# UoB-HPC/neutral

Hardware: AMD Instinct MI355X
Metric: particle-steps/sec (higher is better)
Workload: dtype f64

## Files before the change

neutral_amd/csrc/neutral_abi.hip:

```cpp
#include "neutral_abi_state.h"

#include <utility>

using namespace neutral_abi;


namespace {

struct StageMs {
  double kernel = 0.0, sort = 0.0, stream = 0.0, collide = 0.0, exported = 0.0, exchange = 0.0;
};

struct Step {
  neutral::SolveArgs a = {};
  neutral::StepOptions options;
  bool tiled = false;
  bool decomposed = false;
  bool exchange = false;
  bool pass_export = false;
  bool checked = false;
  State::Store* shard = nullptr;
  neutral::StepCounters hc[2] = {};
  unsigned long long check[8] = {0};
  unsigned ctrl[16] = {0};
// ... 47 lines not shown
      HIP_CHECK(hipEventElapsedTime(&ms, g.ev_start, g.ev_streamed));
    }
    stage.stream += (double)ms;
    HIP_CHECK(hipEventElapsedTime(&ms, g.ev_streamed, g.ev_collected));
    stage.sort += (double)ms;
    HIP_CHECK(hipEventElapsedTime(&ms, g.ev_collected, g.ev_stop));
    stage.collide += (double)ms;
  } else {
    stage.collide += (double)ms;
  }
  HIP_CHECK(hipEventElapsedTime(&ms, g.ev_stop, g.ev_exported));
  stage.exported += (double)ms;
  if (s.exchange) {
    HIP_CHECK(hipEventElapsedTime(&ms, g.ev_exchange_begins, g.ev_exchanged));
    stage.exchange += (double)ms;
  }
}

void export_records_by_id(const Step& s, const int* abort_flag) {
  const neutral::SolveArgs& a = s.a;
  HIP_CHECK(neutral::launch_export_records(
      g.tiled.rec_out, g.tiled.slot_of_id, a.p, a.nparticles, g.stream, abort_flag,
      a.export_skip_long_dead ? neutral::tiled_first_inactive(g.tiled) : nullptr, 0xFFFFFFFFu,
      nullptr, 0, a.export_skip_long_dead != 0));
}

void run_batch(Step& s, const BatchSpec& spec) {
  neutral::SolveArgs& a = s.a;
  HIP_CHECK(hipEventRecord(g.ev_start, g.stream));
  if (s.tiled) {
    HIP_CHECK(neutral::launch_solve_tiled(a, s.options, g.tiled, g.stream, spec.plan, spec.first_pass,
                                          spec.first_sort_timed ? g.ev_sorted : nullptr, g.ev_streamed,
                                          g.ev_collected, &s.passes, spec.split));
  } else {
    HIP_CHECK(neutral::launch_solve(a, s.options, g.variant, g.stream));
  }
  HIP_CHECK(hipEventRecord(g.ev_stop, g.stream));
  if (s.exchange) {
    exchange_step(a, s.tiled);
  } else {
    tallies_to_caller(a);
  }
  if (spec.split) {
    HIP_CHECK(neutral::launch_split_export(a, g.tiled, *spec.split, g.ev_collected));
    HIP_CHECK(hipStreamWaitEvent(g.stream, g.ev_split_done, 0));
  } else if (s.pass_export && !s.decomposed) {
    export_records_by_id(s, spec.guarded ? a.abort_flag : nullptr);
// ... 668 lines not shown
```

neutral_amd/csrc/neutral_history.h:

```cpp
#ifndef NEUTRAL_AMD_HISTORY_H
#define NEUTRAL_AMD_HISTORY_H

#include "neutral_device.h"
#include "neutral_kernels.h"

namespace neutral {

constexpr unsigned kMaxEventsPerHistory = 1u << 27;

enum Event : int {
  kEvEnd = 0,
  kEvFacet = 1,
  kEvCollision = 2,
  kEvCensus = 3,
};

struct History {
  double x, y, omega_x, omega_y, energy, weight, dt_to_census, mfp_to_collision;
  int cellx, celly, dead;
  double local_density, micro_s, micro_a, number_density, macro_s, macro_a, speed;
  double energy_deposition;
  double track_length;
  double u_x_inv, u_y_inv, dep_sigma, dep_heat;
  double r_speed, r_cell_mfp;
// ... 434 lines not shown
  h.id = (unsigned)pid;
}

__device__ __forceinline__ void store_particle_view(const History& h, const ParticleView& p,
                                                    int pid) {
  p.x[pid] = h.x;
  p.y[pid] = h.y;
  p.omega_x[pid] = h.omega_x;
  p.omega_y[pid] = h.omega_y;
  p.energy[pid] = h.energy;
  p.weight[pid] = h.weight;
  p.dt_to_census[pid] = h.dt_to_census;
  p.mfp_to_collision[pid] = h.mfp_to_collision;
  p.cellx[pid] = h.cellx;
  p.celly[pid] = h.celly;
  p.dead[pid] = h.dead;
}

__device__ __forceinline__ void store_particle(const History& h, const SolveArgs& a, int pid) {
  store_particle_view(h, a.p, pid);
}

constexpr int kRecStateBits = 3;
constexpr int kRecChanged = (int)0x80000000u;
constexpr unsigned kIdChanged = 0x80000000u;
__device__ __forceinline__ int record_word(int state, unsigned counter) {
  return state | (int)((counter << kRecStateBits) & 0x7FFFFFFFu);
}
__device__ __forceinline__ int record_state(int word) { return word & ((1 << kRecStateBits) - 1); }
__device__ __forceinline__ unsigned record_counter(int word) {
  return ((unsigned)word & 0x7FFFFFFFu) >> kRecStateBits;
}

__device__ __forceinline__ void load_record(History& h, const SolveArgs& a, const ParticleRec& r,
                                            bool keep_changed = false) {
  h.x = r.x;
  h.y = r.y;
  h.omega_x = r.omega_x;
  h.omega_y = r.omega_y;
  h.energy = r.energy;
  h.weight = r.weight;
  h.dt_to_census = r.dt_to_census;
  h.mfp_to_collision = r.mfp_to_collision;
  h.cellx = r.cellx;
  h.celly = r.celly;
  h.dead = 0;
  h.id = r.id | ((keep_changed && (r.dead & kRecChanged)) ? kIdChanged : 0u);
  h.counter = record_counter(r.dead);
}

enum RecState : int {
  kRecIdle = 0,
  kRecDead = 1,
  kRecCollide = 2,
  kRecMigrate = 3,
  kRecEmigrate = 4,
  kRecGone = 5,
};
constexpr int kReachBits = 2;
constexpr unsigned kSummaryTileMask = (1u << (32 - kRecStateBits - kReachBits)) - 1u;

__device__ __forceinline__ unsigned slot_summary(int state, int cellx, int celly, int tiles_x,
                                                 int tile_shift, unsigned reach = 0u) {
  return ((unsigned)state << (32 - kRecStateBits)) |
         (reach << (32 - kRecStateBits - kReachBits)) |
         ((unsigned)((celly >> tile_shift) * tiles_x + (cellx >> tile_shift)) & kSummaryTileMask);
}
__device__ __forceinline__ unsigned summary_reach(unsigned summary) {
  return (summary >> (32 - kRecStateBits - kReachBits)) & ((1u << kReachBits) - 1u);
}

__device__ __forceinline__ unsigned reach_class(double omega_x, double omega_y, int local_cellx,
                                                int local_celly, int tile_shift, int window_cells,
                                                double cells_per_x, double cells_per_y) {
  const int tile = 1 << tile_shift;
  const int margin = (window_cells - tile) >> 1;
  const int fx = local_cellx & (tile - 1);
  const int fy = local_celly & (tile - 1);
  const double to_edge_x = (double)((omega_x >= 0.0) ? (tile - fx + margin) : (fx + 1 + margin));
  const double to_edge_y = (double)((omega_y >= 0.0) ? (tile - fy + margin) : (fy + 1 + margin));
  const double rate_x = fabs(omega_x) * cells_per_x;
  const double rate_y = fabs(omega_y) * cells_per_y;
  const double path = fmin(to_edge_x / rate_x, to_edge_y / rate_y);
  const double facets = path * (rate_x + rate_y);
  const int cls = (int)(facets * (2.0 / (double)window_cells));
  return (unsigned)((cls < 0) ? 0 : ((cls > 3) ? 3 : cls));
}
__device__ __forceinline__ int summary_state(unsigned summary) {
  return (int)(summary >> (32 - kRecStateBits));
}
__device__ __forceinline__ unsigned summary_tile(unsigned summary) {
  return summary & kSummaryTileMask;
}

__device__ __forceinline__ bool outside_domain(const History& h, const SolveArgs& a) {
  return ((unsigned)(h.cellx - a.x_off) >= (unsigned)a.nx) |
         ((unsigned)(h.celly - a.y_off) >= (unsigned)a.ny);
}

typedef unsigned rec_quad __attribute__((ext_vector_type(4)));
constexpr int kRecQuads = kParticleRecBytes / 16;

__device__ __forceinline__ void record_quads(const History& h, int state, rec_quad (&q)[kRecQuads],
                                             bool changed = false) {
  ParticleRec o;
  o.x = h.x;
  o.y = h.y;
  o.omega_x = h.omega_x;
  o.omega_y = h.omega_y;
  o.energy = h.energy;
  o.weight = h.weight;
  o.dt_to_census = h.dt_to_census;
  o.mfp_to_collision = h.mfp_to_collision;
  o.cellx = h.cellx;
  o.celly = h.celly;
  o.id = h.id & ~kIdChanged;
  o.dead = record_word(state, h.counter) | ((changed || (h.id & kIdChanged)) ? kRecChanged : 0);
  __builtin_memcpy(q, &o, kParticleRecBytes);
}

__device__ __forceinline__ void store_record(const History& h, const SolveArgs& a,
                                             ParticleRec& r, int state, bool changed = false) {
  rec_quad q[kRecQuads];
  record_quads(h, state, q, changed);
  rec_quad* dst = (rec_quad*)__builtin_assume_aligned(&r, 16);
#pragma unroll
  for (int k = 0; k < kRecQuads; ++k) {
    dst[k] = q[k];
  }
}

__device__ __forceinline__ void store_record_through(const History& h, const SolveArgs& a,
                                                     ParticleRec& r, int state) {
  rec_quad q[kRecQuads];
  record_quads(h, state, q);
  static_assert(kRecQuads == 5, "five quads");
  asm volatile(
      "global_store_dwordx4 %0, %1, off sc1\n"
      "global_store_dwordx4 %0, %2, off offset:16 sc1\n"
      "global_store_dwordx4 %0, %3, off offset:32 sc1\n"
      "global_store_dwordx4 %0, %4, off offset:48 sc1\n"
      "global_store_dwordx4 %0, %5, off offset:64 sc1\n"
      "s_nop 1"
      :
      : "v"(&r), "v"(q[0]), "v"(q[1]), "v"(q[2]), "v"(q[3]), "v"(q[4])
      : "memory");
}

__device__ __forceinline__ void drain_stores() { asm volatile("s_waitcnt vmcnt(0)" ::: "memory"); }

__device__ __forceinline__ void load_record_through(History& h, const SolveArgs& a,
                                                    const ParticleRec& r, bool keep_changed = false) {
  rec_quad q[kRecQuads];
  asm volatile(
      "global_load_dwordx4 %0, %5, off sc1\n"
      "global_load_dwordx4 %1, %5, off offset:16 sc1\n"
      "global_load_dwordx4 %2, %5, off offset:32 sc1\n"
      "global_load_dwordx4 %3, %5, off offset:48 sc1\n"
      "global_load_dwordx4 %4, %5, off offset:64 sc1\n"
      "s_waitcnt vmcnt(0)"
      : "=&v"(q[0]), "=&v"(q[1]), "=&v"(q[2]), "=&v"(q[3]), "=&v"(q[4])
      : "v"(&r)
      : "memory");
  ParticleRec o;
  __builtin_memcpy(&o, q, kParticleRecBytes);
  load_record(h, a, o, keep_changed);
}

template <typename T>
__device__ __forceinline__ void load_record_through(History& h, const SolveArgs& a,
                                                    const ParticleRec& r, const T* side, T& side_out) {
  static_assert(sizeof(T) == 16, "one quad");
  rec_quad q[kRecQuads];
  rec_quad s;
  asm volatile(
      "global_load_dwordx4 %0, %6, off sc1\n"
      "global_load_dwordx4 %1, %6, off offset:16 sc1\n"
      "global_load_dwordx4 %2, %6, off offset:32 sc1\n"
      "global_load_dwordx4 %3, %6, off offset:48 sc1\n"
      "global_load_dwordx4 %4, %6, off offset:64 sc1\n"
      "global_load_dwordx4 %5, %7, off sc1\n"
      "s_waitcnt vmcnt(0)"
      : "=&v"(q[0]), "=&v"(q[1]), "=&v"(q[2]), "=&v"(q[3]), "=&v"(q[4]), "=&v"(s)
      : "v"(&r), "v"(side)
      : "memory");
  ParticleRec o;
  __builtin_memcpy(&o, q, kParticleRecBytes);
  load_record(h, a, o);
  __builtin_memcpy(&side_out, &s, 16);
// ... 741 lines not shown
```

neutral_amd/csrc/neutral_kernels.h:

```cpp
#ifndef NEUTRAL_AMD_KERNELS_H
#define NEUTRAL_AMD_KERNELS_H

#include <hip/hip_runtime.h>
#include <stdint.h>

namespace neutral {

struct ParticleView {
  double* x;
  double* y;
  double* omega_x;
  double* omega_y;
  double* energy;
  double* weight;
  double* dt_to_census;
  double* mfp_to_collision;
  int* cellx;
  int* celly;
  int* dead;
};

struct alignas(16) ParticleRec {
  double x, y, dt_to_census, mfp_to_collision;
  int cellx, celly;
  unsigned id;
  int dead;
  double omega_x, omega_y, energy, weight;
};
constexpr int kParticleRecBytes = 80;
static_assert(sizeof(ParticleRec) == kParticleRecBytes, "ParticleRec holds 80 bytes");

struct alignas(16) SuspendExtra {
  double energy_deposition;
  unsigned counter;
  unsigned nevents;
};

struct alignas(16) CarriedStart {
  double micro;
  double minus_log_rn0;
};

struct InjectArgs {
  int nparticles;
  uint64_t pid_base;
  int local_nx;
  int local_ny;
  int pad;
  int x_off;
  int y_off;
  double left_off;
  double bottom_off;
  double width;
// ... 223 lines not shown
hipError_t set_step_options_tiled(const StepOptions& o, hipStream_t stream);
hipError_t launch_solve(const SolveArgs& a, const StepOptions& o, int variant, hipStream_t stream);
hipError_t launch_unphysical_values(const double* v, long long n, unsigned long long* out,
                                    hipStream_t stream);
hipError_t launch_tables_check(const double* ks, const double* vs, int ns, const double* ka,
                               const double* va, int na, unsigned long long expect_hash_s,
                               unsigned long long expect_hash_a, int expect_same,
                               int fast_arithmetic, unsigned long long* out4,
                               hipStream_t stream);


size_t tiled_lds_bytes(const SolveArgs& a, const StepOptions& o, const TiledArgs& t);
hipError_t launch_import_records(const ParticleView& p, ParticleRec* rec, unsigned* info,
                                 unsigned* slot_of_id, unsigned* ids, int tiles_x, int tile_shift,
                                 int x_off, int y_off, int n, hipStream_t stream);
hipError_t launch_refresh_micro(const SolveArgs& a, const TiledArgs& t, hipStream_t stream);
bool tiled_uses_carried(const SolveArgs& a, const TiledArgs& t);
hipError_t launch_export_records(const ParticleRec* rec, const unsigned* slot_of_id,
                                 const ParticleView& p, int n, hipStream_t stream,
                                 const int* abort_flag = nullptr,
                                 const unsigned* first_inactive = nullptr,
                                 unsigned final_from = 0xFFFFFFFFu,
                                 const unsigned* skip_ids = nullptr, int max_blocks = 0,
                                 bool partial_ok = false);
struct SplitExport {
  bool on;
  hipStream_t side;
  hipEvent_t done;
  ParticleView p;
  int skip_long_dead;
};
const unsigned* tiled_first_inactive(const TiledArgs& t);
hipError_t launch_emigrant_count(const TiledArgs& t, int n, const DomainGrid& d, unsigned* counts,
                                 hipStream_t stream);
hipError_t launch_emigrant_pack(const TiledArgs& t, int n, const DomainGrid& d,
                                const unsigned* offset, unsigned* cursor, ParticleRec* send,
                                unsigned* free_slots, unsigned* nfree, hipStream_t stream);
hipError_t launch_immigrant_append(const TiledArgs& t, const ParticleRec* recv, int nrecv,
                                   int first_slot, int x_off, int y_off,
                                   const unsigned* free_slots, int nfree, int reuse,
                                   hipStream_t stream);
hipError_t launch_compact_records(const TiledArgs& t, int n, unsigned* cursor, hipStream_t stream);
hipError_t launch_import_by_slot(const ParticleView& p, const unsigned* keys, const TiledArgs& t,
                                 int x_off, int y_off, int n, hipStream_t stream);
hipError_t launch_export_by_slot(const ParticleRec* rec, const ParticleView& p, unsigned* keys,
                                 int n, hipStream_t stream);
int tiled_tile_shift(int nx, int ny, int nparticles, bool with_flux);
// ... 56 lines not shown
```

neutral_amd/csrc/neutral_kernels.hip:

```cpp
#include "neutral_kernels.h"

#include "neutral_device.h"
#include "neutral_history.h"
#include "neutral_inject.h"
#include "neutral_step_options.h"
#include "neutral_wave.h"

#include <type_traits>

namespace neutral {

constexpr int kBlock = 256;

#define NEUTRAL_COLD_ARGS(a) (kQueue ? cold_args() : (a))


__global__ __launch_bounds__(kBlock) void inject_kernel(InjectArgs a) {
  const int kk = blockIdx.x * kBlock + threadIdx.x;
  if (kk >= a.nparticles) {
    return;
  }
  inject_slot(a, kk, 0, 1.0);
}

// ... 237 lines not shown
  static_assert(sizeof(SolveArgs) % 4 == 0, "SolveArgs is read back word by word");
  union {
    SolveArgs a;
    unsigned w[sizeof(SolveArgs) / 4];
  } u;
#if defined(__HIP_DEVICE_COMPILE__)
  typedef const __attribute__((address_space(4))) unsigned* KernargWords;
  KernargWords p = (KernargWords)__builtin_amdgcn_kernarg_segment_ptr();
  asm volatile("" : "+s"(p));
#pragma unroll
  for (unsigned i = 0; i < sizeof(SolveArgs) / 4; ++i) {
    u.w[i] = p[i];
  }
#else
  __builtin_memset(&u, 0, sizeof(u));
#endif
  return u.a;
}

template <bool kQueue, bool kCarriesMicro = false>
__device__ __forceinline__ void put_back(const History& h, const SolveArgs& a, int pid) {
  if (kQueue) {
    const int state = h.dead ? kRecDead : kRecIdle;
    store_record(h, a, a.rec[pid], state, true);
    a.slot_info[pid] = slot_summary(state, h.cellx - a.x_off, h.celly - a.y_off, a.tiles_x,
                                    a.tile_shift);
    if (kCarriesMicro && a.carried) {
      a.carried[pid].micro = h.micro_s;
    }
    if (a.export_view) {
      const ParticleView* pv = a.export_view;
      asm volatile("" : "+s"(pv));
      store_particle_view(h, *pv, (int)h.id);
    }

  } else {
    store_particle(h, a, pid);
  }
}


template <bool kSameTables, bool kQueue, bool kFlux, bool kChecked, unsigned kScores = 0>
__global__ __launch_bounds__(kBlock, kQueue ? ((kSameTables && !kFlux && !kChecked) ? 4 : 3)
                                             : 3)
void history_regroup_kernel(SolveArgs a) {
  constexpr bool kCollisions = (kScores & kScoreCollisions) != 0;
  constexpr bool kRoulette = (kScores & kScoreRoulette) != 0;
// ... 430 lines not shown
          break;
        }
      }
      if (kQueue) {
        w_ncollisions += (unsigned long long)inner * (unsigned)n_collide;
        if (collides_here) {
          h.nevents += inner;
          if (h.nevents > kMaxEventsPerHistory && want != kWantRefill) {
            atomicAdd(&a.counters->aborted, 1u);
            h.ev = kEvEnd;
            want = kWantStream;
          }
        }
      }
      if (slice_ends) {
        slice = 0;
        const bool out = (want == kWantCollide);
        const unsigned long long m_out = __ballot(out);
        StealWork* const sw = cold_args().steal;
        unsigned readers = __hip_atomic_load(&sw->ring_readers[gw], __ATOMIC_RELAXED, __HIP_MEMORY_SCOPE_AGENT);
        if (out) {
          const SolveArgs c = NEUTRAL_COLD_ARGS(a);
          flush_collision_scores(h, c, tally);
          store_record(h, c, c.rec[pid], kRecCollide);
          SuspendExtra x;
          x.energy_deposition = h.energy_deposition;
          x.counter = h.counter;
          x.nevents = h.nevents;
          c.susp[pid] = x;
          if (kFlux) {
            __hip_atomic_store(&c.susp_track[pid], h.track_length, __ATOMIC_RELAXED, __HIP_MEMORY_SCOPE_AGENT);
          }
          if (kCurrent) {
            double* const pending = d_options.current.susp + 2 * (size_t)pid;
            __hip_atomic_store(&pending[0], h.current_x, __ATOMIC_RELAXED, __HIP_MEMORY_SCOPE_AGENT);
            __hip_atomic_store(&pending[1], h.current_y, __ATOMIC_RELAXED, __HIP_MEMORY_SCOPE_AGENT);
          }
        }
        while (wave_uniform(readers) != 0u) {
          __builtin_amdgcn_s_sleep(1);
          readers = __hip_atomic_load(&sw->ring_readers[gw], __ATOMIC_RELAXED, __HIP_MEMORY_SCOPE_AGENT);
        }
        if (out) {
          __hip_atomic_store(ring_slot(ring_tail + lane_rank(m_out)), (unsigned)pid | kRequeued, __ATOMIC_RELAXED,
                             __HIP_MEMORY_SCOPE_AGENT);
          want = kWantRefill;
        }
        const int n_out = __popcll(m_out);
        w_requeued += (unsigned)n_out;
        drained = false;
        drain_stores();
        unsigned waiting_before = 0;
        if ((threadIdx.x & 63) == 0) {
          waiting_before = (unsigned)atomicAdd(&sw->ring_ctl[gw], (unsigned long long)n_out);
        }
        ring_count = (int)wave_uniform(waiting_before) + n_out;
        ring_tail += n_out;
        ring_tail = (ring_tail >= share) ? ring_tail - share : ring_tail;
      }
    } else {
      if (want == kWantStream) {
        const SolveArgs c = NEUTRAL_COLD_ARGS(a);
        if (h.ev == kEvFacet) {
          nfacets++;
          cross_facet<kChecked>(h, c, tally);
          if (kQueue && c.decomposed && outside_domain(h, c)) {
            store_record(h, c, c.rec[pid], kRecEmigrate);
            c.slot_info[pid] = slot_summary(kRecEmigrate, 0, 0, c.tiles_x, c.tile_shift);
            atomicAdd(c.emigrants, 1u);
            want = kWantRefill;
          } else {
            next_event(true);
            want = (h.ev == kEvCollision) ? kWantCollide : kWantStream;
          }
        } else {
          if (h.ev == kEvCensus) {
            ncensus++;
            census<kChecked>(h, c, tally);
          }
          flush_collision_scores(h, c, tally);
          put_back<kQueue, kSameTables>(h, c, pid);
          want = kWantRefill;
        }
      }
    }
  }
  flush_counters(a, nprocessed, nfacets, ncollisions, ncensus);
  if ((threadIdx.x & 63) == 0) {
    if (w_ncollisions) atomicAdd(&a.counters->ncollisions, w_ncollisions);
    if (w_requeued) atomicAdd(&a.counters->nrequeued, (unsigned long long)w_requeued);
// ... 503 lines not shown
```

neutral_amd/csrc/neutral_tiled.hip:

```cpp
#include <cstdlib>
#include <cstring>
#include <type_traits>

#include "neutral_kernels.h"

#include "neutral_device.h"
#include "neutral_history.h"
#include "neutral_step_options.h"
#include "neutral_wave.h"

namespace neutral {

#ifndef NEUTRAL_STREAM_BLOCK
#define NEUTRAL_STREAM_BLOCK 1024
#endif
constexpr int kStreamBlock = NEUTRAL_STREAM_BLOCK;
constexpr int kChunkParticlesMax = 32768;
constexpr int kChunkParticlesMin = 1024;
constexpr int kStreamRefillMin = 56;
constexpr int kStreamRepeat = 64;
constexpr int kStreamRepeatOnePass = 128;
#ifdef NEUTRAL_NO_CARRIED_START
constexpr bool kCarriedStart = false;
#else
// ... 292 lines not shown
        }
      }
    }
  }
}

__global__ __launch_bounds__(kSortBlock) void import_records_kernel(ParticleView p, ParticleRec* rec,
                                                                    unsigned* info,
                                                                    unsigned* slot_of_id,
                                                                    unsigned* ids, int tiles_x,
                                                                    int tile_shift, int x_off,
                                                                    int y_off, int n) {
  const int i = blockIdx.x * kSortBlock + threadIdx.x;
  if (i < n) {
    ParticleRec r;
    r.x = p.x[i];
    r.y = p.y[i];
    r.omega_x = p.omega_x[i];
    r.omega_y = p.omega_y[i];
    r.energy = p.energy[i];
    r.weight = p.weight[i];
    r.dt_to_census = p.dt_to_census[i];
    r.mfp_to_collision = p.mfp_to_collision[i];
    r.cellx = p.cellx[i];
    r.celly = p.celly[i];
    r.id = (unsigned)i;
    r.dead = p.dead[i];
    rec[i] = r;
    slot_of_id[i] = (unsigned)i;
    ids[i] = (unsigned)i;
    info[i] = slot_summary(r.dead ? kRecDead : kRecIdle, r.cellx - x_off, r.celly - y_off, tiles_x,
                           tile_shift);
  }
}

__global__ __launch_bounds__(kSortBlock) void refresh_micro_kernel(SolveArgs a, TiledArgs t) {
  const long long i = (long long)blockIdx.x * kSortBlock + threadIdx.x;
  if (i >= t.sort_end) {
    return;
  }
  const int state = summary_state(t.info_in[i]);
  if (state == kRecDead || state == kRecGone) {
    return;
  }
  const double energy = t.rec_in[i].energy;
  const int ind = cs_bracket(a.scatter_keys, a.scatter_n, energy);
  t.carried_in[i].micro = a.checked ? cs_interpolate<true>(a.scatter_keys, a.scatter_values, ind, energy)
                            : cs_interpolate<false>(a.scatter_keys, a.scatter_values, ind, energy);
}

__global__ __launch_bounds__(kSortBlock) void export_records_kernel(const ParticleRec* rec,
                                                                    const unsigned* slot_of_id,
                                                                    ParticleView p, int n,
                                                                    const int* abort_flag,
                                                                    const unsigned* first_inactive,
                                                                    unsigned final_from,
                                                                    const unsigned* skip_ids,
                                                                    int partial_ok) {
  if (abort_flag && *abort_flag) {
    return;
  }
  for (long long kk = (long long)blockIdx.x * kSortBlock + threadIdx.x; kk < n; kk += (long long)gridDim.x * kSortBlock) {
    const int k = (int)kk;
    if (skip_ids && ((skip_ids[k >> 5] >> (k & 31)) & 1u)) {
      continue;
    }
    const unsigned slot = slot_of_id[k];
    if (slot >= (first_inactive ? *first_inactive : final_from)) {
      continue;
    }
    const rec_quad* const q = (const rec_quad*)__builtin_assume_aligned(&rec[slot], 16);
    ParticleRec r;
    rec_quad* const rq = (rec_quad*)&r;
    rq[0] = q[0];
    rq[1] = q[1];
    rq[2] = q[2];
    __builtin_nontemporal_store(r.x, &p.x[k]);
    __builtin_nontemporal_store(r.y, &p.y[k]);
    __builtin_nontemporal_store(r.dt_to_census, &p.dt_to_census[k]);
    __builtin_nontemporal_store(r.mfp_to_collision, &p.mfp_to_collision[k]);
    __builtin_nontemporal_store(r.cellx, &p.cellx[k]);
    __builtin_nontemporal_store(r.celly, &p.celly[k]);
    if (!partial_ok || (r.dead & kRecChanged)) {
      rq[3] = q[3];
      rq[4] = q[4];
      __builtin_nontemporal_store(r.omega_x, &p.omega_x[k]);
      __builtin_nontemporal_store(r.omega_y, &p.omega_y[k]);
      __builtin_nontemporal_store(r.energy, &p.energy[k]);
      __builtin_nontemporal_store(r.weight, &p.weight[k]);
      __builtin_nontemporal_store((record_state(r.dead) == kRecDead) ? 1 : 0, &p.dead[k]);
    }
  }
}

__global__ __launch_bounds__(1024) void tile_chunks_kernel(TiledArgs t) {
  __shared__ unsigned s_chunks[1024];
  constexpr int kStagedOffsets = 8192;
  __shared__ unsigned s_offset[kStagedOffsets + 2];
  const int tid = threadIdx.x;
  const bool staged = t.nsort + 1 <= kStagedOffsets;
  if (staged) {
    for (int i = tid; i <= t.nsort + 1; i += 1024) {
      s_offset[i] = t.tile_offset[i];
    }
    __syncthreads();
  }
  const unsigned* offset = staged ? s_offset : t.tile_offset;
  const unsigned nactive = offset[t.nsort];
// ... 525 lines not shown
              unsigned spins = 0;
              do {
                src = __hip_atomic_load(place, __ATOMIC_RELAXED, __HIP_MEMORY_SCOPE_AGENT);
              } while (src == kQueueEmpty && ++spins < (1u << 22));
            } else {
              src = t.order[mine];
            }
            if (src >= (unsigned)a.nparticles) {
              atomicAdd(&a.counters->aborted, 1u);
              ended = true;
            } else {
            pid = fresh ? mine : (int)src;
            double micro = 0.0, minus_log_rn0 = 0.0;
            if (kCarried) {
              const CarriedStart cs = fresh ? t.carried_in[src] : t.carried_out[src];
              micro = cs.micro;
              minus_log_rn0 = cs.minus_log_rn0;
            }
            bool bad_load = false;
            if (from_queue || (queues && !fresh)) {
              load_record_through(h, a, t.rec_out[src], true);
              if (from_queue) {
                const int want_tile = ((h.celly - a.y_off) >> t.tile_shift) * t.tiles_x + ((h.cellx - a.x_off) >> t.tile_shift);
                bad_load = (want_tile != chunk_tile) | (!kDomain && (h.id & ~kIdChanged) >= (unsigned)a.nparticles);
              }
            } else {
              load_record(h, a, fresh ? t.rec_in[src] : t.rec_out[src], !fresh);
            }
            if (fresh) {
              t.id_out[pid] = h.id;
              if (!kDomain && t.slots_by_id) {
                t.slot_of_id[h.id] = (unsigned)pid;
              }
              if (kCarried) {
                t.carried_out[pid].micro = micro;
              }
            }
            if (bad_load) {
              atomicAdd(&a.counters->aborted, 1u);
              ended = true;
            } else {
            if (kCarried) {
              if (fresh) {
                prologue_carried<kChecked>(h, a, micro, minus_log_rn0, uniform_window, window_density);
              } else {
                resume_carried<kChecked>(h, a, micro, uniform_window, window_density);
              }
            } else if (fresh) {
              prologue<kSameTables, kChecked>(h, a, ix);
            } else {
              resume<kSameTables, kChecked>(h, a, ix);
            }
            if (!kDomain) {
              h.counter = 1;
            }
            h.plain_div = 0;
            refresh_speed_reciprocal<kChecked>(h);
            refresh_mfp_reciprocal<kChecked>(h);
            h.dep_rate = deposit_rate(h, a);
// ... 83 lines not shown
            if (!((lx < (unsigned)kW) & (ly < (unsigned)kW)) && far_to_go(h, t)) {
              park = kRecMigrate;
            }
          }
          nfacets += (unsigned)crossed;
          h.nevents += (unsigned)crossed;
          if (!windowed && budget_on && park == kRecIdle && h.ev == kEvFacet &&
              h.nevents >= kUnwindowedBudget) {
            const double ahead = h.speed * h.dt_to_census;
            if (ahead * (fabs(h.omega_x) * t.cells_per_x + fabs(h.omega_y) * t.cells_per_y) >
                kMigrateMinFacets) {
              park = kRecMigrate;
            }
          }
          if (h.nevents > kMaxEventsPerHistory && h.ev == kEvFacet && park == kRecIdle) {
            atomicAdd(&a.counters->aborted, 1u);
            h.ev = kEvEnd;
          }
          PHASE(3);
        } else {
          if (h.ev == kEvCensus) {
            census_streamed<kChecked>(h, a, tally);
          }
          store_record(h, a, t.rec_out[pid], kRecIdle);
          t.info_out[pid] = slot_summary(
              kRecIdle, h.cellx - a.x_off, h.celly - a.y_off, t.tiles_x, t.tile_shift,
              t.reach_classes > 1 ? reach_class(h.omega_x, h.omega_y, h.cellx - a.x_off,
                                                h.celly - a.y_off, t.tile_shift, kW, t.cells_per_x,
                                                t.cells_per_y)
                                  : 0u);
          has = false;
          ended = true;
          did_census = (h.ev == kEvCensus);
          PHASE(6);
        }
      }
      bool queued = false;
      const bool hop = queues && park == kRecMigrate;
      const unsigned long long m_hop = __ballot(hop);
      if (m_hop != 0ull) {
        int dest = 0;
        if (hop) {
          dest = ((h.celly - a.y_off) >> t.tile_shift) * t.tiles_x + ((h.cellx - a.x_off) >> t.tile_shift);
          if ((unsigned)dest >= (unsigned)t.ntiles || (unsigned)pid >= (unsigned)a.nparticles) {
            atomicAdd(&a.counters->aborted, 1u);
            dest = 0;
          }
          store_record_through(h, a, t.rec_out[(unsigned)pid < (unsigned)a.nparticles ? pid : 0], kRecMigrate);
        }
        int leader = -1;
        unsigned rank = 0, group = 0;
        unsigned long long todo = m_hop;
        while (todo != 0ull) {
          const int l = __builtin_ctzll(todo);
          const int tile_l = __builtin_amdgcn_readlane(dest, l);
          const unsigned long long same = __ballot(hop && dest == tile_l);
          if (hop && dest == tile_l) {
            leader = l;
            rank = (unsigned)lane_rank(same);
            group = (unsigned)__popcll(same);
          }
          todo &= ~same;
        }
        drain_stores();
        unsigned base = 0;
        if (hop && leader == (int)(threadIdx.x & 63)) {
          base = atomicAdd(&t.queue_tail[dest], group);
        }
        base = (unsigned)__shfl((int)base, leader < 0 ? 0 : leader, 64);
        if (hop) {
          const unsigned place = base + rank;
          if (place < qcap) {
            __hip_atomic_store(t.queue_entries + ((size_t)dest * qcap + (size_t)place), (unsigned)pid,
                               __ATOMIC_RELAXED, __HIP_MEMORY_SCOPE_AGENT);
            queued = true;
            has = false;
          }
        }
        w_hops += (unsigned)__popcll(__ballot(queued));
        w_overflows += (unsigned)__popcll(__ballot(hop && !queued));
      }
      if (park != kRecIdle && !queued) {
        if (!hop) {
          store_record(h, a, t.rec_out[pid], park);
        }
        t.info_out[pid] = slot_summary(
            park, h.cellx - a.x_off, h.celly - a.y_off, t.tiles_x, t.tile_shift,
            (t.reach_classes > 1 && park == kRecMigrate)
                ? reach_class(h.omega_x, h.omega_y, h.cellx - a.x_off, h.celly - a.y_off,
                              t.tile_shift, kW, t.cells_per_x, t.cells_per_y)
                : 0u);
        has = false;
        ended = true;
      }
      PHASE(7);
      w_ended += (unsigned)__popcll(__ballot(ended));
      w_migrants += (unsigned)__popcll(__ballot(park == kRecMigrate && !queued));
      if (kDomain) {
        w_emigrants += (unsigned)__popcll(__ballot(park == kRecEmigrate));
      }
      w_census += (unsigned)__popcll(__ballot(did_census));
    }
  }
  PHASE(0);
  PHASE_REPORT
  if ((threadIdx.x & 63) == 0 && w_migrants) {
    atomicAdd(&t.ctrl[kCtrlMigrants], w_migrants);
// ... 29 lines not shown
    if ((threadIdx.x & 63) == 0) {
      if (w_processed) atomicAdd(&a.counters->nprocessed, (unsigned long long)w_processed);
      if (wf) atomicAdd(&a.counters->nfacets, (unsigned long long)wf);
      if (w_census) atomicAdd(&a.counters->ncensus, (unsigned long long)w_census);
    }
  }
  clock_stamp_end(a.counters);
}


__device__ __forceinline__ int owner_rank(const DomainGrid& d, int cellx, int celly) {
  int rx = cellx / d.bx;
  int ry = celly / d.by;
  rx = (rx < 0) ? 0 : ((rx >= d.px) ? d.px - 1 : rx);
  ry = (ry < 0) ? 0 : ((ry >= d.py) ? d.py - 1 : ry);
  return ry * d.px + rx;
}

__global__ __launch_bounds__(kSortBlock) void emigrant_count_kernel(const ParticleRec* rec,
                                                                    const unsigned* info, int n,
                                                                    DomainGrid d, unsigned* counts) {
  const int i = blockIdx.x * kSortBlock + threadIdx.x;
  if (i < n && summary_state(info[i]) == kRecEmigrate) {
    atomicAdd(&counts[owner_rank(d, rec[i].cellx, rec[i].celly)], 1u);
  }
}

__global__ __launch_bounds__(kSortBlock) void emigrant_pack_kernel(ParticleRec* rec, unsigned* info,
                                                                   int n, DomainGrid d,
                                                                   const unsigned* offset,
                                                                   unsigned* cursor,
                                                                   ParticleRec* send, int tiles_x,
                                                                   int tile_shift,
                                                                   unsigned* free_slots,
                                                                   unsigned* nfree) {
  const int i = blockIdx.x * kSortBlock + threadIdx.x;
  if (i < n && summary_state(info[i]) == kRecEmigrate) {
    ParticleRec r = rec[i];
    const int dest = owner_rank(d, r.cellx, r.celly);
    const unsigned k = atomicAdd(&cursor[dest], 1u);
    free_slots[atomicAdd(nfree, 1u)] = (unsigned)i;
    const unsigned counter = record_counter(r.dead);
    r.dead = record_word(kRecMigrate, counter);
    send[offset[dest] + k] = r;
    rec[i].dead = record_word(kRecGone, 0u);
    info[i] = slot_summary(kRecGone, 0, 0, tiles_x, tile_shift);
  }
}

__global__ __launch_bounds__(kSortBlock) void immigrant_append_kernel(const ParticleRec* recv,
                                                                      int nrecv, ParticleRec* rec,
                                                                      unsigned* info, unsigned* ids,
                                                                      int first_slot, int x_off,
                                                                      int y_off, int tiles_x,
                                                                      int tile_shift,
                                                                      unsigned* migrants,
                                                                      const unsigned* free_slots,
                                                                      int nfree, int reuse) {
  const int j = blockIdx.x * kSortBlock + threadIdx.x;
  if (j == 0) {
    atomicAdd(migrants, (unsigned)nrecv);
  }
  if (j < nrecv) {
    const ParticleRec r = recv[j];
    const int slot = (j < reuse) ? (int)free_slots[nfree - 1 - j] : first_slot + (j - reuse);
    rec[slot] = r;
    ids[slot] = r.id;
    info[slot] = slot_summary(kRecMigrate, r.cellx - x_off, r.celly - y_off, tiles_x, tile_shift);
  }
}

__global__ __launch_bounds__(kSortBlock) void compact_records_kernel(
    const ParticleRec* rec, const unsigned* info, const unsigned* ids, int n, ParticleRec* rec_to,
    unsigned* info_to, unsigned* ids_to, unsigned* cursor) {
  const int i = blockIdx.x * kSortBlock + threadIdx.x;
  const bool keep = i < n && summary_state(info[i]) != kRecGone;
  const unsigned long long m = __ballot(keep);
  unsigned base = 0;
  if ((threadIdx.x & 63) == 0 && m) {
    base = atomicAdd(cursor, (unsigned)__popcll(m));
  }
  base = __builtin_amdgcn_readfirstlane(base);
  if (keep) {
    const unsigned j = base + (unsigned)lane_rank(m);
    rec_to[j] = rec[i];
    info_to[j] = info[i];
    ids_to[j] = ids[i];
  }
}

__global__ __launch_bounds__(kSortBlock) void import_by_slot_kernel(ParticleView p,
                                                                    const unsigned* keys,
                                                                    ParticleRec* rec, unsigned* info,
                                                                    unsigned* ids, int tiles_x,
                                                                    int tile_shift, int x_off,
                                                                    int y_off, int n) {
  const int i = blockIdx.x * kSortBlock + threadIdx.x;
  if (i < n) {
    ParticleRec r;
    r.x = p.x[i];
    r.y = p.y[i];
    r.omega_x = p.omega_x[i];
    r.omega_y = p.omega_y[i];
    r.energy = p.energy[i];
    r.weight = p.weight[i];
    r.dt_to_census = p.dt_to_census[i];
    r.mfp_to_collision = p.mfp_to_collision[i];
    r.cellx = p.cellx[i];
    r.celly = p.celly[i];
    r.id = keys[i];
    r.dead = p.dead[i] ? kRecDead : kRecIdle;
    rec[i] = r;
    ids[i] = r.id;
    info[i] = slot_summary(p.dead[i] ? kRecDead : kRecIdle, r.cellx - x_off, r.celly - y_off,
                           tiles_x, tile_shift);
  }
}

__global__ __launch_bounds__(kSortBlock) void export_by_slot_kernel(const ParticleRec* rec,
                                                                    ParticleView p, unsigned* keys,
                                                                    int n) {
  const int k = blockIdx.x * kSortBlock + threadIdx.x;
  if (k < n) {
    const ParticleRec r = rec[k];
    p.x[k] = r.x;
    p.y[k] = r.y;
    p.omega_x[k] = r.omega_x;
    p.omega_y[k] = r.omega_y;
    p.energy[k] = r.energy;
    p.weight[k] = r.weight;
    p.dt_to_census[k] = r.dt_to_census;
    p.mfp_to_collision[k] = r.mfp_to_collision;
    p.cellx[k] = r.cellx;
    p.celly[k] = r.celly;
    p.dead[k] = (record_state(r.dead) == kRecDead) ? 1 : 0;
    keys[k] = r.id;
  }
}

hipError_t launch_emigrant_count(const TiledArgs& t, int n, const DomainGrid& d, unsigned* counts,
                                 hipStream_t stream) {
  if (n > 0) {
    hipLaunchKernelGGL(emigrant_count_kernel, dim3((n + kSortBlock - 1) / kSortBlock),
                       dim3(kSortBlock), 0, stream, t.rec_out, t.info_out, n, d, counts);
  }
  return hipGetLastError();
}

hipError_t launch_emigrant_pack(const TiledArgs& t, int n, const DomainGrid& d,
                                const unsigned* offset, unsigned* cursor, ParticleRec* send,
                                unsigned* free_slots, unsigned* nfree, hipStream_t stream) {
  if (n > 0) {
    hipLaunchKernelGGL(emigrant_pack_kernel, dim3((n + kSortBlock - 1) / kSortBlock),
                       dim3(kSortBlock), 0, stream, t.rec_out, t.info_out, n, d, offset, cursor,
                       send, t.tiles_x, t.tile_shift, free_slots, nfree);
    (void)hipMemsetAsync(&t.ctrl[kCtrlEmigrants], 0, sizeof(unsigned), stream);
  }
// ... 112 lines not shown
                       dim3(kSortBlock), 0, stream, p, rec, info, slot_of_id, ids, tiles_x, tile_shift,
                       x_off, y_off, n);
  }
  return hipGetLastError();
}

hipError_t launch_refresh_micro(const SolveArgs& a, const TiledArgs& t, hipStream_t stream) {
  if (t.sort_end > 0) {
    hipLaunchKernelGGL(refresh_micro_kernel, dim3((t.sort_end + kSortBlock - 1) / kSortBlock),
                       dim3(kSortBlock), 0, stream, a, t);
  }
  return hipGetLastError();
}

bool tiled_uses_carried(const SolveArgs& a, const TiledArgs& t) {
  return kCarriedStart && a.same_tables && !a.decomposed && !t.queue_entries && t.carried_in &&
         t.carried_out;
}

hipError_t launch_export_records(const ParticleRec* rec, const unsigned* slot_of_id,
                                 const ParticleView& p, int n, hipStream_t stream,
                                 const int* abort_flag, const unsigned* first_inactive,
                                 unsigned final_from, const unsigned* skip_ids, int max_blocks,
                                 bool partial_ok) {
  if (n > 0) {
    int grid = (n + kSortBlock - 1) / kSortBlock;
    grid = (max_blocks > 0 && grid > max_blocks) ? max_blocks : grid;
    hipLaunchKernelGGL(export_records_kernel, dim3(grid), dim3(kSortBlock), 0, stream, rec,
                       slot_of_id, p, n, abort_flag, first_inactive, final_from, skip_ids, partial_ok ? 1 : 0);
  }
  return hipGetLastError();
}

const unsigned* tiled_first_inactive(const TiledArgs& t) { return &t.ctrl[kCtrlFirstInactive]; }

static hipError_t enqueue_stream_pass(const SolveArgs& a, const StepOptions& o, TiledArgs& t, int pass,
                                      int cus, size_t lds, hipStream_t stream, hipEvent_t after_sort) {
  t.pass = pass;
  t.allow_migrate = (pass + 1 < kMaxStreamPasses) ? 1 : 0;
  const int grid_n = (a.nparticles + kSortBlock - 1) / kSortBlock;
  const int grid_seg = t.sort_end > 0 ? (t.sort_end + kSortSegment - 1) / kSortSegment : 1;
  const int nbins = t.nsort + 1;
  const size_t lds_bins = (nbins <= kSortLdsBins) ? sizeof(unsigned) * (size_t)nbins : 0;
  hipLaunchKernelGGL(tile_count_kernel, dim3(grid_seg), dim3(kSortBlock), lds_bins, stream, a, t);
  hipLaunchKernelGGL(tile_scan_kernel, dim3(1), dim3(1024), 0, stream, t);
  hipLaunchKernelGGL(tile_scatter_kernel, dim3(grid_seg), dim3(kSortBlock), 2 * lds_bins, stream, a,
                     t);
  hipLaunchKernelGGL(tile_chunks_kernel, dim3(1), dim3(1024), 0, stream, t);
  if (pass == 0) {
    hipLaunchKernelGGL(copy_inactive_kernel, dim3(grid_n < 8192 ? grid_n : 8192), dim3(kSortBlock), 0, stream,
                       a, t);
    if (after_sort) {
// ... 87 lines not shown
  c.rec = t.rec_out;
  c.slot_info = t.info_out;
  c.tiles_x = t.tiles_x;
  c.tile_shift = t.tile_shift;
  c.susp = t.susp;
  c.susp_track = t.susp_track;
  c.carried = t.carried ? t.carried_out : nullptr;
  c.steal = t.steal;
  c.emigrants = &t.ctrl[kCtrlEmigrants];
  if (t.fine_index && c.same_tables) {
    c.scatter_index = t.fine_index;
    c.scatter_index_n = t.fine_index_n;
    c.scatter_index_base = t.fine_index_base;
    c.index_shift = t.fine_index_shift;
  }
  return launch_solve(c, o, kVariantEventSorted, stream);
}

hipError_t launch_split_export(const SolveArgs& a, const TiledArgs& t, const SplitExport& split,
                               hipEvent_t after_collect) {
  (void)hipStreamWaitEvent(split.side, after_collect, 0);
  (void)launch_export_records(t.rec_out, t.slot_of_id, split.p, a.nparticles, split.side, a.abort_flag,
                              split.skip_long_dead ? &t.ctrl[kCtrlFirstInactive] : nullptr, 0xFFFFFFFFu,
                              t.susp_ids, 0, split.skip_long_dead != 0);
  (void)hipEventRecord(split.done, split.side);
  return hipGetLastError();
}


}
```

Measured before the change: 145.3 billion.

## Reorder particle record so census-kept particles export from a two-quad head

Reorders the 80-byte ParticleRec so position, collision clock, low 16-bit cell halves and the state word sit in the first 32 bytes, with the census clock and high cell halves in the third quad. A new census-kept flag in the state bits marks particles that started and ended the step at census without a collision. For those, the export kernel reads only the head and writes x, y, mfp and cells, skipping dt_to_census (already zero) and the rest of the record. This trims record reads and SoA writes in the export pass, at the cost of split cell encoding, renumbered record states and extra flag bookkeeping in the solve kernels.

```diff
diff --git a/neutral_amd/csrc/neutral_abi.hip b/neutral_amd/csrc/neutral_abi.hip
--- a/neutral_amd/csrc/neutral_abi.hip
+++ b/neutral_amd/csrc/neutral_abi.hip
@@ -93,7 +93,8 @@
   HIP_CHECK(neutral::launch_export_records(
       g.tiled.rec_out, g.tiled.slot_of_id, a.p, a.nparticles, g.stream, abort_flag,
       a.export_skip_long_dead ? neutral::tiled_first_inactive(g.tiled) : nullptr, 0xFFFFFFFFu,
-      nullptr, 0, a.export_skip_long_dead != 0));
+      nullptr, 0, a.export_skip_long_dead != 0,
+      neutral::record_head_holds_cells(a.global_nx, a.global_ny)));
 }
 
 void run_batch(Step& s, const BatchSpec& spec) {
diff --git a/neutral_amd/csrc/neutral_history.h b/neutral_amd/csrc/neutral_history.h
--- a/neutral_amd/csrc/neutral_history.h
+++ b/neutral_amd/csrc/neutral_history.h
@@ -480,18 +480,36 @@
 }
 
 constexpr int kRecStateBits = 3;
+enum RecState : int {
+  kRecIdle = 0,
+  kRecDead = 1,
+  kRecCollide = 2,
+  kRecMigrate = 3,
+  kRecEmigrate = 5,
+  kRecGone = 6,
+};
 constexpr int kRecChanged = (int)0x80000000u;
 constexpr unsigned kIdChanged = 0x80000000u;
+constexpr int kRecCensusKept = 1 << (kRecStateBits - 1);
+constexpr unsigned kIdFromCensus = 0x40000000u;
+constexpr unsigned kIdFlags = kIdChanged | kIdFromCensus;
+constexpr int kRecCounterBits = 31 - kRecStateBits;
+static_assert(kRecCounterBits == 28 && kMaxEventsPerHistory <= (1u << (kRecCounterBits - 1)),
+              "the record's RNG counter holds what a history can draw before the watchdog ends it");
 __device__ __forceinline__ int record_word(int state, unsigned counter) {
   return state | (int)((counter << kRecStateBits) & 0x7FFFFFFFu);
 }
 __device__ __forceinline__ int record_state(int word) { return word & ((1 << kRecStateBits) - 1); }
+static_assert((kRecIdle | kRecCensusKept) != kRecEmigrate && (kRecIdle | kRecCensusKept) != kRecGone &&
+                  (kRecMigrate | kRecCensusKept) != kRecEmigrate &&
+                  (kRecMigrate | kRecCensusKept) != kRecGone && kRecGone < (1 << kRecStateBits),
+              "a flagged state is no other state's number");
 __device__ __forceinline__ unsigned record_counter(int word) {
   return ((unsigned)word & 0x7FFFFFFFu) >> kRecStateBits;
 }
 
 __device__ __forceinline__ void load_record(History& h, const SolveArgs& a, const ParticleRec& r,
-                                            bool keep_changed = false) {
+                                            bool keep_flags = false) {
   h.x = r.x;
   h.y = r.y;
   h.omega_x = r.omega_x;
@@ -500,21 +518,21 @@
   h.weight = r.weight;
   h.dt_to_census = r.dt_to_census;
   h.mfp_to_collision = r.mfp_to_collision;
-  h.cellx = r.cellx;
-  h.celly = r.celly;
+  h.cellx = record_cellx(r);
+  h.celly = record_celly(r);
   h.dead = 0;
-  h.id = r.id | ((keep_changed && (r.dead & kRecChanged)) ? kIdChanged : 0u);
+  h.id = r.id | ((keep_flags && (r.dead & kRecChanged)) ? kIdChanged : 0u) |
+         ((keep_flags && record_state(r.dead) == (kRecMigrate | kRecCensusKept)) ? kIdFromCensus : 0u);
   h.counter = record_counter(r.dead);
 }
 
-enum RecState : int {
-  kRecIdle = 0,
-  kRecDead = 1,
-  kRecCollide = 2,
-  kRecMigrate = 3,
-  kRecEmigrate = 4,
-  kRecGone = 5,
-};
+__device__ __forceinline__ void note_census_start(History& h) {
+  h.id |= (__double_as_longlong(h.dt_to_census) == 0ll) ? kIdFromCensus : 0u;
+}
+__device__ __forceinline__ bool began_at_census(const History& h) {
+  return (h.id & kIdFromCensus) != 0u;
+}
+
 constexpr int kReachBits = 2;
 constexpr unsigned kSummaryTileMask = (1u << (32 - kRecStateBits - kReachBits)) - 1u;
 
@@ -560,7 +578,8 @@
 constexpr int kRecQuads = kParticleRecBytes / 16;
 
 __device__ __forceinline__ void record_quads(const History& h, int state, rec_quad (&q)[kRecQuads],
-                                             bool changed = false) {
+                                             bool changed, bool census_kept) {
+  const bool flagged = census_kept && ((state == kRecIdle) | (state == kRecMigrate));
   ParticleRec o;
   o.x = h.x;
   o.y = h.y;
@@ -570,17 +589,18 @@
   o.weight = h.weight;
   o.dt_to_census = h.dt_to_census;
   o.mfp_to_collision = h.mfp_to_collision;
-  o.cellx = h.cellx;
-  o.celly = h.celly;
-  o.id = h.id & ~kIdChanged;
-  o.dead = record_word(state, h.counter) | ((changed || (h.id & kIdChanged)) ? kRecChanged : 0);
+  record_set_cell(o, h.cellx, h.celly);
+  o.id = h.id & ~kIdFlags;
+  o.dead = record_word(state | (flagged ? kRecCensusKept : 0), h.counter) |
+           ((changed || (h.id & kIdChanged)) ? kRecChanged : 0);
   __builtin_memcpy(q, &o, kParticleRecBytes);
 }
 
 __device__ __forceinline__ void store_record(const History& h, const SolveArgs& a,
-                                             ParticleRec& r, int state, bool changed = false) {
+                                             ParticleRec& r, int state, bool changed,
+                                             bool census_kept) {
   rec_quad q[kRecQuads];
-  record_quads(h, state, q, changed);
+  record_quads(h, state, q, changed, census_kept);
   rec_quad* dst = (rec_quad*)__builtin_assume_aligned(&r, 16);
 #pragma unroll
   for (int k = 0; k < kRecQuads; ++k) {
@@ -589,9 +609,10 @@
 }
 
 __device__ __forceinline__ void store_record_through(const History& h, const SolveArgs& a,
-                                                     ParticleRec& r, int state) {
+                                                     ParticleRec& r, int state, bool changed,
+                                                     bool census_kept) {
   rec_quad q[kRecQuads];
-  record_quads(h, state, q);
+  record_quads(h, state, q, changed, census_kept);
   static_assert(kRecQuads == 5, "five quads");
   asm volatile(
       "global_store_dwordx4 %0, %1, off sc1\n"
@@ -608,7 +629,7 @@
 __device__ __forceinline__ void drain_stores() { asm volatile("s_waitcnt vmcnt(0)" ::: "memory"); }
 
 __device__ __forceinline__ void load_record_through(History& h, const SolveArgs& a,
-                                                    const ParticleRec& r, bool keep_changed = false) {
+                                                    const ParticleRec& r, bool keep_flags = false) {
   rec_quad q[kRecQuads];
   asm volatile(
       "global_load_dwordx4 %0, %5, off sc1\n"
@@ -622,7 +643,7 @@
       : "memory");
   ParticleRec o;
   __builtin_memcpy(&o, q, kParticleRecBytes);
-  load_record(h, a, o, keep_changed);
+  load_record(h, a, o, keep_flags);
 }
 
 template <typename T>
diff --git a/neutral_amd/csrc/neutral_kernels.h b/neutral_amd/csrc/neutral_kernels.h
--- a/neutral_amd/csrc/neutral_kernels.h
+++ b/neutral_amd/csrc/neutral_kernels.h
@@ -2,6 +2,7 @@
 #define NEUTRAL_AMD_KERNELS_H
 
 #include <hip/hip_runtime.h>
+#include <stddef.h>
 #include <stdint.h>
 
 namespace neutral {
@@ -21,14 +22,47 @@
 };
 
 struct alignas(16) ParticleRec {
-  double x, y, dt_to_census, mfp_to_collision;
-  int cellx, celly;
+  double x, y, mfp_to_collision;
+  unsigned cells_lo;
+  int dead;
+  double dt_to_census;
   unsigned id;
-  int dead;
+  unsigned cells_hi;
   double omega_x, omega_y, energy, weight;
 };
 constexpr int kParticleRecBytes = 80;
+constexpr int kRecHeadBytes = 32;
+constexpr int kRecHeadCells = 1 << 16;
 static_assert(sizeof(ParticleRec) == kParticleRecBytes, "ParticleRec holds 80 bytes");
+static_assert(offsetof(ParticleRec, dead) + sizeof(int) == kRecHeadBytes &&
+                  offsetof(ParticleRec, x) < kRecHeadBytes && offsetof(ParticleRec, y) < kRecHeadBytes &&
+                  offsetof(ParticleRec, mfp_to_collision) < kRecHeadBytes &&
+                  offsetof(ParticleRec, cells_lo) < kRecHeadBytes,
+              "the head: position, collision clock, low cell halves, state word");
+static_assert(offsetof(ParticleRec, dt_to_census) == kRecHeadBytes &&
+                  offsetof(ParticleRec, cells_hi) + sizeof(unsigned) == kRecHeadBytes + 16,
+              "the third quad: census clock, id, high cell halves");
+static_assert(offsetof(ParticleRec, omega_x) == 48, "what only a collision or a reflection changes: last");
+
+__host__ __device__ __forceinline__ int record_cellx(const ParticleRec& r) {
+  return (int)((r.cells_lo & 0xFFFFu) | (r.cells_hi << 16));
+}
+__host__ __device__ __forceinline__ int record_celly(const ParticleRec& r) {
+  return (int)((r.cells_lo >> 16) | (r.cells_hi & 0xFFFF0000u));
+}
+__host__ __device__ __forceinline__ void record_set_cell(ParticleRec& r, int cellx, int celly) {
+  r.cells_lo = ((unsigned)cellx & 0xFFFFu) | ((unsigned)celly << 16);
+  r.cells_hi = ((unsigned)cellx >> 16) | ((unsigned)celly & 0xFFFF0000u);
+}
+__host__ __device__ __forceinline__ int record_head_cellx(const ParticleRec& r) {
+  return (int)(r.cells_lo & 0xFFFFu);
+}
+__host__ __device__ __forceinline__ int record_head_celly(const ParticleRec& r) {
+  return (int)(r.cells_lo >> 16);
+}
+inline bool record_head_holds_cells(int global_nx, int global_ny) {
+  return global_nx <= kRecHeadCells && global_ny <= kRecHeadCells;
+}
 
 struct alignas(16) SuspendExtra {
   double energy_deposition;
@@ -298,7 +332,7 @@
                                  const unsigned* first_inactive = nullptr,
                                  unsigned final_from = 0xFFFFFFFFu,
                                  const unsigned* skip_ids = nullptr, int max_blocks = 0,
-                                 bool partial_ok = false);
+                                 bool partial_ok = false, bool head_cells = false);
 struct SplitExport {
   bool on;
   hipStream_t side;
diff --git a/neutral_amd/csrc/neutral_kernels.hip b/neutral_amd/csrc/neutral_kernels.hip
--- a/neutral_amd/csrc/neutral_kernels.hip
+++ b/neutral_amd/csrc/neutral_kernels.hip
@@ -283,7 +283,7 @@
 __device__ __forceinline__ void put_back(const History& h, const SolveArgs& a, int pid) {
   if (kQueue) {
     const int state = h.dead ? kRecDead : kRecIdle;
-    store_record(h, a, a.rec[pid], state, true);
+    store_record(h, a, a.rec[pid], state, true, false);
     a.slot_info[pid] = slot_summary(state, h.cellx - a.x_off, h.celly - a.y_off, a.tiles_x,
                                     a.tile_shift);
     if (kCarriesMicro && a.carried) {
@@ -760,7 +760,7 @@
         if (out) {
           const SolveArgs c = NEUTRAL_COLD_ARGS(a);
           flush_collision_scores(h, c, tally);
-          store_record(h, c, c.rec[pid], kRecCollide);
+          store_record(h, c, c.rec[pid], kRecCollide, false, false);
           SuspendExtra x;
           x.energy_deposition = h.energy_deposition;
           x.counter = h.counter;
@@ -803,7 +803,7 @@
           nfacets++;
           cross_facet<kChecked>(h, c, tally);
           if (kQueue && c.decomposed && outside_domain(h, c)) {
-            store_record(h, c, c.rec[pid], kRecEmigrate);
+            store_record(h, c, c.rec[pid], kRecEmigrate, false, false);
             c.slot_info[pid] = slot_summary(kRecEmigrate, 0, 0, c.tiles_x, c.tile_shift);
             atomicAdd(c.emigrants, 1u);
             want = kWantRefill;
diff --git a/neutral_amd/csrc/neutral_tiled.hip b/neutral_amd/csrc/neutral_tiled.hip
--- a/neutral_amd/csrc/neutral_tiled.hip
+++ b/neutral_amd/csrc/neutral_tiled.hip
@@ -338,15 +338,15 @@
     r.weight = p.weight[i];
     r.dt_to_census = p.dt_to_census[i];
     r.mfp_to_collision = p.mfp_to_collision[i];
-    r.cellx = p.cellx[i];
-    r.celly = p.celly[i];
+    const int cellx = p.cellx[i];
+    const int celly = p.celly[i];
+    record_set_cell(r, cellx, celly);
     r.id = (unsigned)i;
-    r.dead = p.dead[i];
+    r.dead = p.dead[i] ? kRecDead : kRecIdle;
     rec[i] = r;
     slot_of_id[i] = (unsigned)i;
     ids[i] = (unsigned)i;
-    info[i] = slot_summary(r.dead ? kRecDead : kRecIdle, r.cellx - x_off, r.celly - y_off, tiles_x,
-                           tile_shift);
+    info[i] = slot_summary(r.dead, cellx - x_off, celly - y_off, tiles_x, tile_shift);
   }
 }
 
@@ -372,7 +372,7 @@
                                                                     const unsigned* first_inactive,
                                                                     unsigned final_from,
                                                                     const unsigned* skip_ids,
-                                                                    int partial_ok) {
+                                                                    int partial_ok, int head_cells) {
   if (abort_flag && *abort_flag) {
     return;
   }
@@ -388,18 +388,27 @@
     const rec_quad* const q = (const rec_quad*)__builtin_assume_aligned(&rec[slot], 16);
     ParticleRec r;
     rec_quad* const rq = (rec_quad*)&r;
+    static_assert(kRecHeadBytes == 32, "the head is two quads");
     rq[0] = q[0];
     rq[1] = q[1];
-    rq[2] = q[2];
+    const bool changed = !partial_ok || (r.dead & kRecChanged);
     __builtin_nontemporal_store(r.x, &p.x[k]);
     __builtin_nontemporal_store(r.y, &p.y[k]);
-    __builtin_nontemporal_store(r.dt_to_census, &p.dt_to_census[k]);
     __builtin_nontemporal_store(r.mfp_to_collision, &p.mfp_to_collision[k]);
-    __builtin_nontemporal_store(r.cellx, &p.cellx[k]);
-    __builtin_nontemporal_store(r.celly, &p.celly[k]);
-    if (!partial_ok || (r.dead & kRecChanged)) {
+    if (head_cells && !changed && record_state(r.dead) == (kRecIdle | kRecCensusKept)) {
+      __builtin_nontemporal_store(record_head_cellx(r), &p.cellx[k]);
+      __builtin_nontemporal_store(record_head_celly(r), &p.celly[k]);
+      continue;
+    }
+    rq[2] = q[2];
+    if (changed) {
       rq[3] = q[3];
       rq[4] = q[4];
+    }
+    __builtin_nontemporal_store(r.dt_to_census, &p.dt_to_census[k]);
+    __builtin_nontemporal_store(record_cellx(r), &p.cellx[k]);
+    __builtin_nontemporal_store(record_celly(r), &p.celly[k]);
+    if (changed) {
       __builtin_nontemporal_store(r.omega_x, &p.omega_x[k]);
       __builtin_nontemporal_store(r.omega_y, &p.omega_y[k]);
       __builtin_nontemporal_store(r.energy, &p.energy[k]);
@@ -971,7 +980,7 @@
               load_record_through(h, a, t.rec_out[src], true);
               if (from_queue) {
                 const int want_tile = ((h.celly - a.y_off) >> t.tile_shift) * t.tiles_x + ((h.cellx - a.x_off) >> t.tile_shift);
-                bad_load = (want_tile != chunk_tile) | (!kDomain && (h.id & ~kIdChanged) >= (unsigned)a.nparticles);
+                bad_load = (want_tile != chunk_tile) | (!kDomain && (h.id & ~kIdFlags) >= (unsigned)a.nparticles);
               }
             } else {
               load_record(h, a, fresh ? t.rec_in[src] : t.rec_out[src], !fresh);
@@ -984,6 +993,7 @@
               if (kCarried) {
                 t.carried_out[pid].micro = micro;
               }
+              note_census_start(h);
             }
             if (bad_load) {
               atomicAdd(&a.counters->aborted, 1u);
@@ -1113,7 +1123,7 @@
           if (h.ev == kEvCensus) {
             census_streamed<kChecked>(h, a, tally);
           }
-          store_record(h, a, t.rec_out[pid], kRecIdle);
+          store_record(h, a, t.rec_out[pid], kRecIdle, false, h.ev == kEvCensus && began_at_census(h));
           t.info_out[pid] = slot_summary(
               kRecIdle, h.cellx - a.x_off, h.celly - a.y_off, t.tiles_x, t.tile_shift,
               t.reach_classes > 1 ? reach_class(h.omega_x, h.omega_y, h.cellx - a.x_off,
@@ -1137,7 +1147,8 @@
             atomicAdd(&a.counters->aborted, 1u);
             dest = 0;
           }
-          store_record_through(h, a, t.rec_out[(unsigned)pid < (unsigned)a.nparticles ? pid : 0], kRecMigrate);
+          store_record_through(h, a, t.rec_out[(unsigned)pid < (unsigned)a.nparticles ? pid : 0], kRecMigrate,
+                               false, began_at_census(h));
         }
         int leader = -1;
         unsigned rank = 0, group = 0;
@@ -1173,7 +1184,7 @@
       }
       if (park != kRecIdle && !queued) {
         if (!hop) {
-          store_record(h, a, t.rec_out[pid], park);
+          store_record(h, a, t.rec_out[pid], park, false, began_at_census(h));
         }
         t.info_out[pid] = slot_summary(
             park, h.cellx - a.x_off, h.celly - a.y_off, t.tiles_x, t.tile_shift,
@@ -1249,7 +1260,7 @@
                                                                     DomainGrid d, unsigned* counts) {
   const int i = blockIdx.x * kSortBlock + threadIdx.x;
   if (i < n && summary_state(info[i]) == kRecEmigrate) {
-    atomicAdd(&counts[owner_rank(d, rec[i].cellx, rec[i].celly)], 1u);
+    atomicAdd(&counts[owner_rank(d, record_cellx(rec[i]), record_celly(rec[i]))], 1u);
   }
 }
 
@@ -1264,7 +1275,7 @@
   const int i = blockIdx.x * kSortBlock + threadIdx.x;
   if (i < n && summary_state(info[i]) == kRecEmigrate) {
     ParticleRec r = rec[i];
-    const int dest = owner_rank(d, r.cellx, r.celly);
+    const int dest = owner_rank(d, record_cellx(r), record_celly(r));
     const unsigned k = atomicAdd(&cursor[dest], 1u);
     free_slots[atomicAdd(nfree, 1u)] = (unsigned)i;
     const unsigned counter = record_counter(r.dead);
@@ -1293,7 +1304,7 @@
     const int slot = (j < reuse) ? (int)free_slots[nfree - 1 - j] : first_slot + (j - reuse);
     rec[slot] = r;
     ids[slot] = r.id;
-    info[slot] = slot_summary(kRecMigrate, r.cellx - x_off, r.celly - y_off, tiles_x, tile_shift);
+    info[slot] = slot_summary(kRecMigrate, record_cellx(r) - x_off, record_celly(r) - y_off, tiles_x, tile_shift);
   }
 }
 
@@ -1333,14 +1344,14 @@
     r.weight = p.weight[i];
     r.dt_to_census = p.dt_to_census[i];
     r.mfp_to_collision = p.mfp_to_collision[i];
-    r.cellx = p.cellx[i];
-    r.celly = p.celly[i];
+    const int cellx = p.cellx[i];
+    const int celly = p.celly[i];
+    record_set_cell(r, cellx, celly);
     r.id = keys[i];
     r.dead = p.dead[i] ? kRecDead : kRecIdle;
     rec[i] = r;
     ids[i] = r.id;
-    info[i] = slot_summary(p.dead[i] ? kRecDead : kRecIdle, r.cellx - x_off, r.celly - y_off,
-                           tiles_x, tile_shift);
+    info[i] = slot_summary(r.dead, cellx - x_off, celly - y_off, tiles_x, tile_shift);
   }
 }
 
@@ -1358,8 +1369,8 @@
     p.weight[k] = r.weight;
     p.dt_to_census[k] = r.dt_to_census;
     p.mfp_to_collision[k] = r.mfp_to_collision;
-    p.cellx[k] = r.cellx;
-    p.celly[k] = r.celly;
+    p.cellx[k] = record_cellx(r);
+    p.celly[k] = record_celly(r);
     p.dead[k] = (record_state(r.dead) == kRecDead) ? 1 : 0;
     keys[k] = r.id;
   }
@@ -1518,12 +1529,13 @@
                                  const ParticleView& p, int n, hipStream_t stream,
                                  const int* abort_flag, const unsigned* first_inactive,
                                  unsigned final_from, const unsigned* skip_ids, int max_blocks,
-                                 bool partial_ok) {
+                                 bool partial_ok, bool head_cells) {
   if (n > 0) {
     int grid = (n + kSortBlock - 1) / kSortBlock;
     grid = (max_blocks > 0 && grid > max_blocks) ? max_blocks : grid;
     hipLaunchKernelGGL(export_records_kernel, dim3(grid), dim3(kSortBlock), 0, stream, rec,
-                       slot_of_id, p, n, abort_flag, first_inactive, final_from, skip_ids, partial_ok ? 1 : 0);
+                       slot_of_id, p, n, abort_flag, first_inactive, final_from, skip_ids, partial_ok ? 1 : 0,
+                       (partial_ok && head_cells) ? 1 : 0);
   }
   return hipGetLastError();
 }
@@ -1657,7 +1669,8 @@
   (void)hipStreamWaitEvent(split.side, after_collect, 0);
   (void)launch_export_records(t.rec_out, t.slot_of_id, split.p, a.nparticles, split.side, a.abort_flag,
                               split.skip_long_dead ? &t.ctrl[kCtrlFirstInactive] : nullptr, 0xFFFFFFFFu,
-                              t.susp_ids, 0, split.skip_long_dead != 0);
+                              t.susp_ids, 0, split.skip_long_dead != 0,
+                              record_head_holds_cells(a.global_nx, a.global_ny));
   (void)hipEventRecord(split.done, split.side);
   return hipGetLastError();
 }
```

After: 142.9 billion. 0.983x the previous value.
